# immaaane/dealii-stfem

Measured on AMD Instinct MI355X. Metric: space-time DoF/s per vmult (3D heat, Q4 space x cG(2) time); achieved HBM GB/s, higher is better.
Workload: dtype f64; 1 GPU; 3D heat, Q4 x cG(2), 72x72x72 cells Cartesian slab mesh, 48275138 space-time DoFs = BASELINE configs[1]; n_blocks=2, cells_per_gpu=373248, partition=z-slabs x1, kernel=st_sweep_pencil<f64>

## Files before the change

### dealii-stfem_amd/__init__.py

```python
import ctypes as C
import os
import subprocess

import numpy as np

_HERE = os.path.dirname(os.path.abspath(__file__))
LIB_PATH = os.path.join(_HERE, "libstfem_hip.so")
HEADER_PATH = os.path.join(os.path.dirname(_HERE), "include", "stfem.h")

CGP, DG = 0, 1


class StfemError(RuntimeError):
    def __init__(self, status, what=""):
        self.status = status
        msg = lib().stfem_strerror(status).decode()
        hip = lib().stfem_last_hip_error().decode()
        super().__init__(f"{what}: {msg} ({status})" + (f" [{hip}]" if hip else ""))


def build(force=False):
    args = ["make", "-C", os.path.join(_HERE, "csrc"), "-j8"]
    if force:
        args.append("-B")
# ... 127 lines not shown
                                        C.POINTER(_vp), _vp]),
    "stfem_stokes_st_vmult_slice_add": (C.c_int, [_vp, C.c_int, C.c_int, C.c_int, _dp, _dp, C.POINTER(_vp),
                                                  _vp, _vp, _vp]),
    "stfem_stokes_last_hip_error": (C.c_char_p, []),
    "stfem_stokes_set_weak_boundaries": (C.c_int, [_vp, C.c_int, C.c_int, C.c_double, C.c_double]),
    "stfem_stokes_n_face_points": (C.c_int64, [_vp]),
    "stfem_stokes_face_points": (C.c_int, [_vp, _dp]),
    "stfem_stokes_nitsche_rhs": (C.c_int, [_vp, _dp, _vp, _vp, _vp]),
    "stfem_stokes_pressure_ctx": (C.c_int, [_vp, C.POINTER(_vp)]),
    "stfem_stokes_pressure_mean_vectors": (C.c_int, [_vp, _dp, _dp, _dp]),
    "stfem_stokes_pressure_quadrature_points": (C.c_int, [_vp, C.c_int, _dp]),
    "stfem_stokes_pressure_difference": (C.c_int, [_vp, C.c_int, _vp, _dp, _dp, _vp]),
    "stfem_stokes_dgp_prolongate": (C.c_int, [_vp, _vp, _vp, _vp, C.c_int, _vp]),
    "stfem_stokes_dgp_restrict": (C.c_int, [_vp, _vp, _vp, _vp, C.c_int, _vp]),
    "stfem_stokes_vanka_create": (C.c_int, [_vp, C.c_int, C.POINTER(C.c_int32), _dp, _dp, C.POINTER(_vp)]),
    "stfem_stokes_vanka_destroy": (None, [_vp]),
    "stfem_stokes_vanka_n_classes": (C.c_int, [_vp]),
    "stfem_stokes_vanka_vmult": (C.c_int, [_vp, C.POINTER(_vp), C.POINTER(_vp), _vp]),
    "stfem_stokes_vanka_step": (C.c_int, [_vp, C.POINTER(_vp), C.c_double, C.c_int, C.POINTER(_vp), _vp]),
    "stfem_stokes_vanka_last_error": (C.c_char_p, []),
    "stfem_strerror": (C.c_char_p, [C.c_int]),
    "stfem_last_hip_error": (C.c_char_p, []),
    "stfem_last_kernel_name": (C.c_char_p, [_vp]),
}


def lib():
    global _lib
    if _lib is None:
        if not os.path.exists(LIB_PATH):
            raise ImportError(f"{LIB_PATH} is missing: run `make -C dealii-stfem_amd/csrc` "
                              "(or __graft_entry__.build()); there is no CPU fallback")
        L = C.CDLL(os.environ.get("STFEM_LIB", LIB_PATH))
        for name, (res, args) in SIGNATURES.items():
            f = getattr(L, name)
            f.restype = res
            f.argtypes = args
        _lib = L
    return _lib


def _p(a):
    return a.ctypes.data_as(_dp)


def _check(status, what):
# ... 170 lines not shown
               "stfem_space_vmult")

    def compute_diagonal(self, mass=None, laplace=None, stream=None):
        d = BlockVector(self, 1)
        _check(lib().stfem_diagonal(self._h,
                                    self.mass_matrix_scaling if mass is None else mass,
                                    self.laplace_matrix_scaling if laplace is None else laplace,
                                    d._h, stream), "stfem_diagonal")
        return d

    def get_matrix_diagonal(self, stream=None):
        return self.compute_diagonal(stream=stream)

    def get_matrix_diagonal_inverse(self, stream=None):
        d = BlockVector(self, 1)
        _check(lib().stfem_diagonal_inverse(self._h, self.mass_matrix_scaling, self.laplace_matrix_scaling,
                                            d._h, stream), "stfem_diagonal_inverse")
        return d

    @property
    def last_kernel_name(self):
        return lib().stfem_last_kernel_name(self._h).decode()


class PreconditionVanka:

    def __init__(self, ctx, Alpha, Beta, neighbour_mask=0, extended=None):
        self.ctx = ctx
        A = np.ascontiguousarray(Alpha, dtype=np.float64)
        B = np.ascontiguousarray(Beta, dtype=np.float64)
        assert A.shape == B.shape and A.shape[0] == A.shape[1]
        h = _vp()
        if extended is not None:
            _check(lib().stfem_vanka_create_partitioned_general(ctx._h, extended._h, A.shape[0], _p(A), _p(B), neighbour_mask, C.byref(h)),
                   "stfem_vanka_create_partitioned_general")
        else:
            _check(lib().stfem_vanka_create_partitioned(ctx._h, A.shape[0], _p(A), _p(B), neighbour_mask, C.byref(h)),
                   "stfem_vanka_create")
        self._h, self.n_blocks = h, A.shape[0]

    def __del__(self):
        if getattr(self, "_h", None) and _lib is not None:
            _lib.stfem_vanka_destroy(self._h)
            self._h = None

    @property
# ... 477 lines not shown
```

### dealii-stfem_amd/csrc/stfem_capi.hip

```cpp
#include "../../include/stfem.h"

#include "host_tables.h"
#include "stfem_internal.h"
#include "stfem_kernels.h"

#include <hip/hip_runtime.h>
#include <dlfcn.h>

#include <algorithm>
#include <cmath>
#include <cstdio>
#include <cstdlib>
#include <cstring>
#include <limits>
#include <new>
#include <string>
#include <vector>

using namespace stfem;

struct Prec64 {
  using real = double;
  using Sweep = f64::SweepParams;
  using Plan = f64::TilePlan;
// ... 150 lines not shown
    const double tol = 1e-13 * std::max({std::abs(up[0] - lo[0]), std::abs(up[1] - lo[1]),
                                         std::abs(up[2] - lo[2]), 1e-300});
    for (int64_t k = 0, o = 0; k < nvz && cart; ++k)
      for (int64_t j = 0; j < nvy && cart; ++j)
        for (int64_t i = 0; i < nvx; ++i, ++o) {
          if (std::abs(v[3 * o] - (lo[0] + c->h[0] * i)) > tol ||
              std::abs(v[3 * o + 1] - (lo[1] + c->h[1] * j)) > tol ||
              std::abs(v[3 * o + 2] - (lo[2] + c->h[2] * k)) > tol) {
            cart = false;
            break;
          }
        }
    c->cartesian = cart;
    c->vertices.assign(v, v + 3 * nv);
  }
  if (const char *v = getenv("STFEM_VARIANT")) c->variant = std::string(v) == "atomic" ? 1 : (std::string(v) == "tile" ? 2 : 0);
  auto env_int = [](const char *name, int dflt) { const char *e = getenv(name); return e ? atoi(e) : dflt; };
  c->env_tile_lz = env_int("STFEM_TILE_LZ", 0);
  c->env_exp = env_int("STFEM_EXP", 0);
  c->env_stagger = env_int("STFEM_STAGGER", 0);
  c->env_stagger_div = std::max(1, env_int("STFEM_STAGGER_DIV", 256));
  c->env_pencil_ty = env_int("STFEM_PENCIL_TY", 0);
  c->env_pencil_lz = env_int("STFEM_PENCIL_LZ", 0);
  c->env_timeline = getenv("STFEM_TIMELINE");
  if (hipMalloc(&c->d_scratch, sizeof(double) * (256 + 8 * 512)) != hipSuccess) {
    delete c;
    return STFEM_ERR_OUT_OF_MEMORY;
  }
  *out = c;
  return STFEM_OK;
}

void stfem_ctx_destroy(stfem_ctx *c)
{
  if (!c) return;
  (void)hipSetDevice(c->device);
  for (void *&p : c->d_coef)
    if (p) (void)hipFree(p);
  if (c->d_scratch) (void)hipFree(c->d_scratch);
  if (c->d_halo) (void)hipFree(c->d_halo);
  if (c->d_vertices) (void)hipFree(c->d_vertices);
  if (c->d_rule) (void)hipFree(c->d_rule);
  if (c->d_metric) (void)hipFree(c->d_metric);
  if (c->d_timeline) (void)hipFree(c->d_timeline);
  if (c->d_work) (void)hipFree(c->d_work);
  delete c;
}

int64_t stfem_n_dofs(const stfem_ctx *c) { return c ? c->ndofs : 0; }
int64_t stfem_n_cells(const stfem_ctx *c) { return c ? c->ncells : 0; }
int stfem_n_dofs_1d(const stfem_ctx *c, int32_t nd[3])
{
  if (!c || !nd) return STFEM_ERR_INVALID_ARGUMENT;
  for (int d = 0; d < 3; ++d) nd[d] = c->nd[d];
  return STFEM_OK;
}
int stfem_is_cartesian(const stfem_ctx *c) { return c && c->cartesian ? 1 : 0; }
int stfem_ctx_precision(const stfem_ctx *c) { return c ? c->prec : -1; }
const char *stfem_last_kernel_name(const stfem_ctx *c) { return c ? c->last_kernel : ""; }

int stfem_set_coefficient(stfem_ctx *c, int which, int layout, const double *host)
{
  if (!c || which < 0 || which > 1 || layout < 0 || layout > 2) return STFEM_ERR_INVALID_ARGUMENT;
  HIP_TRY(hipSetDevice(c->device));
  if (c->d_coef[which]) {
    HIP_TRY(hipFree(c->d_coef[which]));
    c->d_coef[which] = nullptr;
  }
// ... 162 lines not shown
  tp.nty = (c->nc[1] + tp.rows - 1) / tp.rows;
  const int ncz = c->nc[2];
  int ntc = 1;
  if (c->env_tile_lz > 0) {
    const int lz = std::max(1, std::min(ncz, c->env_tile_lz));
    ntc = (ncz + lz - 1) / lz;
  } else {
    (void)nbm;
    const int wpc = std::max(2, resident);
    const int64_t slots = int64_t(c->n_cu > 0 ? c->n_cu : 256) * wpc;
    const int64_t columns = int64_t((tp.ntx + 1) / 2) * tp.nty;
    double best = 1e300;
    for (int n = 1; n <= ncz; ++n) {
      const int64_t rounds = (columns * n + slots - 1) / slots;
      const double cost = double(rounds) * ((ncz + n - 1) / n + 1.0) * (1.0 + 1e-3 * n);
      if (cost < best) { best = cost; ntc = n; }
    }
  }
  tp.ntc = ntc;
  tp.lz = (ncz + ntc - 1) / ntc;
  tp.zp = c->p * tp.lz + 1;
}

template <class PL> static void plan_pencil(const stfem_ctx *c, PL &pp)
{
  pp.ntx = (c->nc[0] + pp.cpw - 2) / (pp.cpw - 1);
  const int cyw = pp.ty * 4;
  pp.ntyw = (c->nc[1] + cyw - 1) / cyw;
  const int ncz = c->nc[2];
  int B = c->env_pencil_lz > 0 ? c->env_pencil_lz : 8;
  B = std::max(B, (ncz + 47) / 48);
  int n = 0, r = ncz;
  pp.zb[0] = 0;
  while (r > 0) {
    const int sz = c->env_pencil_lz < 0 ? std::min(std::max(-c->env_pencil_lz, (ncz + 47) / 48), r)
                                        : std::min(B, std::max(1, (r + 2) / 3));
    r -= sz;
    pp.zb[n + 1] = pp.zb[n] + sz;
    if (n == 62 && r > 0) {
      pp.zb[n + 2] = ncz;
      n += 2;
      r = 0;
      break;
    }
    ++n;
  }
  pp.ntc = n;
  pp.lz = 0;
  for (int q = 0; q < n; ++q) pp.lz = std::max(pp.lz, pp.zb[q + 1] - pp.zb[q]);
  pp.zp = c->p * pp.lz + 1;
}

template <class PR> static int ensure_metric(stfem_ctx *c, bool use_lap, bool use_mass, hipStream_t st)
{
  using real = typename PR::real;
  const int n = c->p + 1;
  const size_t nm = size_t(c->ncells) * 8 * n * n * n;
  const int flags = (use_lap ? 1 : 0) | (use_mass ? 2 : 0);
  if (c->metric_valid && c->metric_flags == flags) return STFEM_OK;
  if (!c->d_vertices) {
    std::vector<double> v = c->vertices;
    if (v.empty()) {
      v.resize(size_t(c->nc[0] + 1) * (c->nc[1] + 1) * (c->nc[2] + 1) * 3);
      size_t o = 0;
      for (int k = 0; k <= c->nc[2]; ++k)
        for (int j = 0; j <= c->nc[1]; ++j)
          for (int i = 0; i <= c->nc[0]; ++i, ++o) {
            v[3 * o] = c->lower[0] + c->h[0] * i;
            v[3 * o + 1] = c->lower[1] + c->h[1] * j;
            v[3 * o + 2] = c->lower[2] + c->h[2] * k;
          }
    }
    std::vector<double> rule(c->tab.xq);
// ... 91 lines not shown
    for (int i0 = 0; i0 < nbi; i0 += panel) {
      const int tj = std::min(panel, nbo - j0), ti = std::min(panel, nbi - i0);
      bool nonzero = false;
      for (int j = 0; j < tj; ++j)
        for (int i = 0; i < ti; ++i) {
          prm.alpha[j * ti + i] = real(a[size_t(j0 + j) * nbi + i0 + i]);
          prm.beta[j * ti + i] = real(b[size_t(j0 + j) * nbi + i0 + i]);
          nonzero = nonzero || prm.alpha[j * ti + i] != real(0) || prm.beta[j * ti + i] != real(0);
        }
      const bool last_panel = i0 + panel >= nbi;
      if (!nonzero && (atomic || add || !first || !last_panel)) continue;
      prm.nbo = tj;
      prm.nbi = ti;
      for (int j = 0; j < tj; ++j) prm.dst[j] = static_cast<real *>(dst->blk[j0 + j]);
      for (int i = 0; i < ti; ++i) prm.src[i] = static_cast<const real *>(src->blk[i0 + i]);
      int rc;
      typename PR::PPlan pp;
      std::memset(&pp, 0, sizeof(pp));
      const int pencil_ty = c->env_pencil_ty;
      if (atomic) {
        rc = PR::atomic(c->p, prm, st);
        c->last_kernel = PR::atomic_name();
      } else if (c->variant == 0 && !general && PR::pencil_geometry(c->p, std::max(tj, ti), pencil_ty, pp) == 0) {
        plan_pencil(c, pp);
        const int nbm = std::max(tj, ti);
        const int nbm_r = nbm <= 4 ? nbm : (nbm <= 6 ? 6 : 8);
        const size_t ntiles = size_t(pp.ntx) * pp.ntyw * pp.ntc;
        const size_t nyh = ntiles * nbm_r * pp.zp * pp.tX, nzh = ntiles * nbm_r * pp.tYW * pp.tX;
        if (nyh + nzh > c->halo_doubles) {
          HIP_TRY(hipStreamSynchronize(st));
          if (c->d_halo) HIP_TRY(hipFree(c->d_halo));
          c->d_halo = nullptr;
          c->halo_doubles = 0;
          if (hipMalloc(&c->d_halo, (nyh + nzh) * sizeof(real)) != hipSuccess) return STFEM_ERR_OUT_OF_MEMORY;
          c->halo_doubles = nyh + nzh;
        }
        pp.yh = static_cast<real *>(c->d_halo);
        pp.zh = pp.yh + nyh;
        pp.add = (add || !first) ? 1 : 0;
        prm.gp = nullptr;
        if constexpr (sizeof(real) == 8) {
          if (c->grad_p && c->p == 2 && tj == 3 && ti == 3 && !pp.add && last_panel && !prm.coef_lap && !prm.coef_mass) {
            prm.gp = c->grad_p;
            prm.gscale = c->grad_scale;
            std::memcpy(prm.gw, c->grad_w, sizeof(prm.gw));
            c->grad_applied = true;
          }
        }
        if (!c->d_work) {
          if (hipMalloc(&c->d_work, 8 * 32 * sizeof(int)) != hipSuccess) return STFEM_ERR_OUT_OF_MEMORY;
          HIP_TRY(hipMemsetAsync(c->d_work, 0, 8 * 32 * sizeof(int), st));
        }
        pp.work = c->d_work;
        pp.grid = 2 * (c->n_cu > 0 ? c->n_cu : 256);
        const size_t ptl_n = ntiles * 4 * pp.lz * pp.ty * 8;
        if (c->env_timeline) {
          if (c->tl_n < ptl_n) {
            if (c->d_timeline) HIP_TRY(hipFree(c->d_timeline));
            c->d_timeline = nullptr;
            if (hipMalloc(&c->d_timeline, ptl_n * sizeof(long long)) != hipSuccess) return STFEM_ERR_OUT_OF_MEMORY;
            c->tl_n = ptl_n;
          }
          HIP_TRY(hipMemsetAsync(c->d_timeline, 0, ptl_n * sizeof(long long), st));
          pp.timeline = c->d_timeline;
        }
        rc = PR::pencil(c->p, prm, pp, st);
        c->last_kernel = PR::pencil_name();
        if (c->env_timeline && rc == 0) {
          HIP_TRY(hipStreamSynchronize(st));
          std::vector<long long> h(ptl_n);
          HIP_TRY(hipMemcpy(h.data(), c->d_timeline, ptl_n * sizeof(long long), hipMemcpyDeviceToHost));
          if (FILE *f = fopen(c->env_timeline, "wb")) {
            const long long hdr[4] = {(long long)ntiles, 4, (long long)pp.lz * pp.ty, 8};
            fwrite(hdr, sizeof(long long), 4, f);
            fwrite(h.data(), sizeof(long long), ptl_n, f);
            fclose(f);
          }
// ... 691 lines not shown
```

### dealii-stfem_amd/csrc/stfem_internal.h

```cpp
#pragma once
#include "../../include/stfem.h"

#include "host_tables.h"

#include <cstdint>
#include <vector>

struct stfem_ctx {
  int p = 0, device = 0, n_cu = 0;
  int nc[3] = {0, 0, 0}, nd[3] = {0, 0, 0};
  int64_t ndofs = 0, ncells = 0;
  int dmask = 0;
  bool cartesian = false;
  double lower[3] = {0, 0, 0}, h[3] = {1, 1, 1};
  stfem::ShapeTables tab;
  std::vector<double> vertices;
  int prec = 0;
  size_t es = sizeof(double);
  void *d_coef[2] = {nullptr, nullptr};
  int coef_layout[2] = {0, 0};
  double *d_scratch = nullptr;
  const char *last_kernel = "";
  void *d_halo = nullptr;
  size_t halo_doubles = 0;
  int variant = 0;
  int env_tile_lz = 0, env_exp = 0, env_stagger = 0, env_stagger_div = 256, env_pencil_ty = 0, env_pencil_lz = 0;
  const char *env_timeline = nullptr;
  int *d_work = nullptr;
  long long *d_timeline = nullptr;
  size_t tl_n = 0;
  double *d_vertices = nullptr, *d_rule = nullptr;
  void *d_metric = nullptr;
  bool metric_valid = false;
  int metric_flags = -1;
  const double *grad_p = nullptr;
  double grad_w[3][2][3][2];
  double grad_scale = 0.0;
  bool grad_applied = false;
};
int stfem_internal_set_gradient(stfem_ctx *c, const double *p, const double (*w)[2][3][2], double scale);

struct stfem_vec {
  stfem_ctx *ctx = nullptr;
  int device = 0;
  int nb = 0;
  bool owns = false;
  std::vector<void *> blk;
};


int stfem_internal_metric(stfem_ctx *c, const void **metric, void *stream);
// ... 9 lines not shown
```

### dealii-stfem_amd/csrc/stfem_kernels_decl.h

```cpp
namespace stfem {
namespace STFEM_NS {

using real_t = STFEM_REAL;

struct SweepParams {
  const real_t *src[MAX_BLOCKS];
  real_t *dst[MAX_BLOCKS];
  real_t alpha[MAX_BLOCKS * MAX_BLOCKS];
  real_t beta[MAX_BLOCKS * MAX_BLOCKS];
  int nbi, nbo;
  int ncx, ncy, ncz;
  int nx, ny, nz;
  int64_t ncells;
  int dmask;
  real_t vol;
  real_t ihx2, ihy2, ihz2;
  const real_t *coef_lap;
  const real_t *coef_mass;
  int experiment;
  real_t eo_Si[EO_N], eo_L[EO_N];
  real_t fd_W[EO_N], fd_lx[8], fd_ly[8], fd_lz[8];
  real_t eo_S[EO_N], eo_Dq[EO_N], eo_DqT[EO_N];
  const real_t *metric;
  const real_t *gp;
  real_t gw[3][2][3][2];
  real_t gscale;
};

struct TilePlan {
  int cw, rows;
  int wx;
  int ntx, nty, ntc;
  int lz;
  int tX, tY, zp;
  real_t *yh, *zh;
  real_t *xl, *xr;
  int add;
  int xcolor;
  int stagger;
  int stagger_div;
  int experiment;
  long long *timeline;
};

struct PencilPlan {
  int cpw, ty;
  int ntx, ntyw, ntc;
  int lz;
  int zb[65];
  int tX, tYW, zp;
  real_t *yh, *zh;
  int add;
  int *work;
  int grid;
  long long *timeline;
};
int pencil_geometry(int p, int nbm, int ty, PencilPlan &plan);
int launch_pencil(int p, const SweepParams &prm, const PencilPlan &plan, void *stream);

int launch_cart_atomic(int p, const SweepParams &prm, void *stream);
const char *cart_atomic_name(int p, int nbm);

struct DiagParams {
  real_t *diag;
  int ncx, ncy, ncz, nx, ny, p, dmask;
  real_t ms, ls;
  real_t vol, ihx2, ihy2, ihz2;
  const real_t *coef_lap, *coef_mass;
  const real_t *metric;
  real_t m1[8], l1[8];
  real_t S[64], D[64];
};
// ... 13 lines not shown
```

### dealii-stfem_amd/csrc/stfem_pencil.hip

```cpp
#include "stfem_core.h"

#include <cstdio>
#include <cstdlib>

#ifndef STFEM_PENCIL_P
#define STFEM_PENCIL_P 0
#endif

namespace stfem {
namespace STFEM_PREC {

namespace {

constexpr int PENCIL_WY = 4;

#ifndef STFEM_PENCIL_EXP
#define STFEM_PENCIL_EXP 0
#endif
constexpr int PEX = STFEM_PENCIL_EXP;

template <typename T> __device__ __forceinline__ void vm_load(T &dst, const T *p)
{
  if constexpr (sizeof(T) == 8) asm volatile("global_load_dwordx2 %0, %1, off" : "=v"(dst) : "v"(p) : "memory");
  else asm volatile("global_load_dword %0, %1, off" : "=v"(dst) : "v"(p) : "memory");
// ... 69 lines not shown
  const int wave = __builtin_amdgcn_readfirstlane(threadIdx.x >> 6);
  real_t *lds = smem + wave * Core::LDS_PER_WAVE;
  real_t *mail_base = smem + WY * Core::LDS_PER_WAVE;
  real_t *mail_out = mail_base + wave * 2 * PG::MAIL;
  const real_t *mail_in = mail_base + (wave - 1) * 2 * PG::MAIL;
  volatile int *flags = reinterpret_cast<volatile int *>(mail_base + (WY - 1) * 2 * PG::MAIL);
  volatile int *prod = flags, *cons = flags + WY;
  volatile int *s_tile = flags + 2 * WY;
  real_t *wtab = const_cast<real_t *>(reinterpret_cast<volatile real_t *>(flags + 2 * WY + 4));
  [[maybe_unused]] real_t *gpt = wtab + PG::WTAB + wave * PG::GPT_WAVE;
  if constexpr (PG::WLDS) {
    for (int e = threadIdx.x; e < NBM * NBM; e += PG::NT) {
      const int j = e / NBM, q = e % NBM;
      const bool ok = j < prm.nbo && q < prm.nbi;
      wtab[2 * e] = ok ? prm.alpha[j * prm.nbi + q] * prm.vol : real_t(0);
      wtab[2 * e + 1] = ok ? prm.beta[j * prm.nbi + q] * prm.vol : real_t(0);
    }
  }
  auto flag_wait = [&](volatile int *f, int target) {
    while (*f < target) __builtin_amdgcn_s_sleep(1);
    asm volatile("" ::: "memory");
  };

  const int ncol = pp.ntx * pp.ntyw;
  unsigned xcc = 0;
  asm volatile("s_getreg_b32 %0, hwreg(HW_REG_XCC_ID)" : "=s"(xcc));
  xcc &= 7;
  for (;;) {
  __syncthreads();
  if (threadIdx.x == 0) {
    int t = -1;
    const int per = ncol / 8, rem = ncol % 8;
    for (int q = 0; q < 8 && t < 0; ++q) {
      const int x = (xcc + q) & 7;
      const int lo = x * per + min(x, rem), n = per + (x < rem ? 1 : 0);
      if (n > 0) {
        const int k = atomicAdd(pp.work + 32 * x, 1);
        if (k < n * pp.ntc) t = (k / n) * ncol + lo + k % n;
      }
    }
    *s_tile = t;
  }
  prod[wave] = 0;
  cons[wave] = 0;
  __syncthreads();
  const int id = __builtin_amdgcn_readfirstlane(*s_tile);
  if (id < 0) break;
  const int tx = id % pp.ntx, tyw = (id / pp.ntx) % pp.ntyw, tc = id / (pp.ntx * pp.ntyw);
  const int wg_tile = id;
  const int wy = tyw * WY + wave;
  const int cx0 = tx * (CPW - 1) - 1, cy0 = wy * TY;
  const int cz0 = pp.zb[tc];
  const int nlay = pp.zb[tc + 1] - cz0;
  const int nslot = min(CPW, prm.ncx - cx0);
  const int ncy_t = max(0, min(TY, prm.ncy - cy0));
  const bool last_x = tx == pp.ntx - 1, last_z = tc == pp.ntc - 1;
  const bool mesh_top = cy0 + TY >= prm.ncy;
  const bool top_mail = !mesh_top && wave < WY - 1;
  const bool top_halo = !mesh_top && wave == WY - 1;
  const bool has_lower = wave > 0;

  const bool lane_ok = lane < PG::ACTIVE;
  const int l = lane_ok ? lane : 0;
  const int i = l % N, c = (l / N) % CPW, blk = l / (N * CPW);
  const int X = P * c + i;
  unsigned lf = 0;
  {
    const bool cell_ok = lane_ok && c < nslot && cx0 + c >= 0 && ncy_t > 0;
    const int cxl = cx0 + (cell_ok ? c : 1);
    const bool out = cell_ok && blk < prm.nbo;
    const bool st = out && c > 0 && (i < P || cxl == prm.ncx - 1);
    const bool xcon = ((prm.dmask & 1) && cxl == 0 && i == 0) || ((prm.dmask & 2) && cxl == prm.ncx - 1 && i == P);
    lf = (cell_ok && blk < prm.nbi ? LF_IN : 0) | (out ? LF_OUT : 0) | (c == nslot - 1 ? LF_LAST : 0) |
         (st ? LF_ST : 0) | (xcon ? LF_XCON : 0);
  }
  const int cx = cx0 + ((lf & (LF_IN | LF_OUT)) ? c : 1);

  [[maybe_unused]] real_t gwx[3] = {real_t(0), real_t(0), real_t(0)}, gWy[N][2], gWz[N][2];
  [[maybe_unused]] int gxv = 0;
// ... 351 lines not shown
    flag_wait(prod + (wave - 1), nlay);
    const real_t *m = mail_in + ((nlay - 1) & 1) * PG::MAIL + lane;
    real_t *d = dst_lane + plane_stride * (int64_t(P) * (nlay - 1));
    real_t v[N];
    STFEM_UNROLL
    for (int z = 0; z < P; ++z) v[z] = pend[z] + m[64 * z];
    v[P] = zfin0 + m[64 * P];
    if (lf & LF_ST) {
      const bool xc = lf & LF_XCON;
      STFEM_UNROLL
      for (int z = 0; z < P; ++z) put(d + plane_stride * z, xc ? real_t(0) : v[z]);
      if (last_z) put(d + plane_stride * P, xc ? real_t(0) : v[P]);
      else (pp.zh + ((int64_t(wg_tile) * NBM + blk) * pp.tYW + P * TY * wave) * pp.tX + X)[0] = xc ? real_t(0) : v[P];
    }
  }
  }
}

template <int P>
__global__ __launch_bounds__(256) void st_pencil_fixup(const SweepParams prm, const PencilPlan pp, int nbm, int cpw, int ty)
{
  const int id = blockIdx.x;
  if (id == 0 && blockIdx.y == 0 && blockIdx.z == 0 && threadIdx.x < 8) pp.work[32 * threadIdx.x] = 0;
  const int tx = id % pp.ntx, tyw = (id / pp.ntx) % pp.ntyw, tc = id / (pp.ntx * pp.ntyw);
  const int has_y = tyw > 0, has_z = tc > 0;
  if (!(has_y | has_z)) return;
  const int cyw = ty * PENCIL_WY;
  const int cx0 = tx * (cpw - 1) - 1, cy0 = tyw * cyw, cz0 = pp.zb[tc];
  const int nslot = min(cpw, prm.ncx - cx0), ncy_t = min(cyw, prm.ncy - cy0);
  const int nlay = pp.zb[tc + 1] - cz0;
  const bool last_x = tx == pp.ntx - 1, last_y = tyw == pp.ntyw - 1, last_z = tc == pp.ntc - 1;
  const int x_begin = P, x_end = P * nslot + (last_x ? 1 : 0);
  const int Yn = P * ncy_t + (last_y ? 1 : 0), Zn = P * nlay + (last_z ? 1 : 0);
  const int lpr = pp.tX <= 16 ? 16 : (pp.tX <= 32 ? 32 : 64), nrg = 256 / lpr;
  const int X = threadIdx.x % lpr, rg = threadIdx.x / lpr;
  if (X < x_begin || X >= x_end) return;
  const int64_t plane_stride = int64_t(prm.nx) * prm.ny;
  const int64_t g0 = int64_t(P) * cx0 + X + int64_t(prm.nx) * (int64_t(P) * cy0) + plane_stride * (int64_t(P) * cz0);
  const int tid_y = id - pp.ntx, tid_z = id - pp.ntx * pp.ntyw, tid_yz = tid_z - pp.ntx;
  const int top_below = has_z ? P * (cz0 - pp.zb[tc - 1]) : 0;
  const int j = blockIdx.y;
  real_t *d = prm.dst[j] + g0;
  const int64_t sy = int64_t(pp.zp) * pp.tX, sz = int64_t(pp.tYW) * pp.tX;
  const real_t *yh_y = pp.yh + (int64_t(tid_y) * nbm + j) * sy + X;
  const real_t *yh_yz = pp.yh + (int64_t(tid_yz) * nbm + j) * sy + X;
  const real_t *zh_z = pp.zh + (int64_t(tid_z) * nbm + j) * sz + X;
  constexpr int U = 4;
  if (has_y && blockIdx.z == 0)
    for (int Z0 = rg + has_z; Z0 < Zn; Z0 += U * nrg) {
      real_t s[U], v[U];
      STFEM_UNROLL
      for (int u = 0; u < U; ++u) {
        const int Z = Z0 + u * nrg;
        s[u] = v[u] = real_t(0);
        if (Z < Zn) {
          s[u] = yh_y[Z * pp.tX];
          v[u] = d[plane_stride * Z];
        }
      }
      STFEM_UNROLL
      for (int u = 0; u < U; ++u) {
        const int Z = Z0 + u * nrg;
        if (Z < Zn) d[plane_stride * Z] = v[u] + s[u];
      }
    }
  if (has_z && blockIdx.z == 1)
    for (int Y0 = rg; Y0 < Yn; Y0 += U * nrg) {
      real_t s[U], v[U];
      STFEM_UNROLL
      for (int u = 0; u < U; ++u) {
        const int Y = Y0 + u * nrg;
        s[u] = v[u] = real_t(0);
        if (Y < Yn) {
          s[u] = zh_z[Y * pp.tX];
          if (Y == 0 && has_y) s[u] += yh_y[0] + yh_yz[top_below * pp.tX];
          v[u] = d[int64_t(prm.nx) * Y];
        }
      }
      STFEM_UNROLL
      for (int u = 0; u < U; ++u) {
        const int Y = Y0 + u * nrg;
        if (Y < Yn) d[int64_t(prm.nx) * Y] = v[u] + s[u];
      }
    }
}

template <int P, int NBM, int TY> int launch_pencil_ty(const SweepParams &prm, const PencilPlan &pp, hipStream_t st)
{
  using PG = PencilGeom<P, NBM, TY>;
  (void)hipGetLastError();
  const bool coef = prm.coef_lap || prm.coef_mass;
  const int nblocks = pp.ntx * pp.ntyw * pp.ntc;
  const int grid = nblocks < pp.grid ? nblocks : pp.grid;
#define STFEM_LAUNCH(AA, CC)                                                                                       \
  do {                                                                                                            \
    static bool lds_set = false;                                                                                  \
    if (!lds_set) {                                                                                               \
      if (hipFuncSetAttribute(reinterpret_cast<const void *>(&st_sweep_pencil<P, NBM, TY, AA, CC>),               \
                              hipFuncAttributeMaxDynamicSharedMemorySize, int(PG::LDS_BYTES)) != hipSuccess)      \
        return -3;                                                                                                \
      lds_set = true;                                                                                             \
    }                                                                                                             \
    hipLaunchKernelGGL((st_sweep_pencil<P, NBM, TY, AA, CC>), dim3(grid), dim3(PG::NT), PG::LDS_BYTES, st, prm, pp); \
  } while (0)
  if constexpr (PG::HAS_GRAD) {
    if (prm.gp) {
      if (pp.add || coef) return -2;
      static bool lds_set = false;
      if (!lds_set) {
        if (hipFuncSetAttribute(reinterpret_cast<const void *>(&st_sweep_pencil<P, NBM, TY, false, false, true>), hipFuncAttributeMaxDynamicSharedMemorySize,
                                int(PG::LDS_BYTES)) != hipSuccess)
          return -3;
        lds_set = true;
      }
      hipLaunchKernelGGL((st_sweep_pencil<P, NBM, TY, false, false, true>), dim3(grid), dim3(PG::NT), PG::LDS_BYTES, st, prm, pp);
    }
  }
  if (PG::HAS_GRAD && prm.gp) {
  } else if (pp.add && coef) STFEM_LAUNCH(true, true);
  else if (pp.add) STFEM_LAUNCH(true, false);
  else if (coef) STFEM_LAUNCH(false, true);
  else STFEM_LAUNCH(false, false);
#undef STFEM_LAUNCH
  const bool sweep_ok = hipGetLastError() == hipSuccess;
  bool fixed_up = false;
  if (sweep_ok && (pp.ntyw > 1 || pp.ntc > 1)) {
    hipLaunchKernelGGL((st_pencil_fixup<P>), dim3(nblocks, prm.nbo, 2), dim3(256), 0, st, prm, pp, NBM, PG::CPW, TY);
    fixed_up = hipGetLastError() == hipSuccess;
    if (!fixed_up) (void)hipMemsetAsync(pp.work, 0, 8 * 32 * sizeof(int), st);
    return fixed_up ? 0 : -3;
  }
  if (hipMemsetAsync(pp.work, 0, 8 * 32 * sizeof(int), st) != hipSuccess || !sweep_ok) return -3;
  return 0;
}

constexpr int pencil_ty(int p, int nbm) { return (p == 4 && nbm == 3) ? 1 : ((p <= 2 && nbm <= 4) ? 4 : 2); }
constexpr int pencil_ty_default(int p, int nbm) { return pencil_ty(p, nbm); }

template <int P, int NBM> int launch_pencil_t(const SweepParams &prm, const PencilPlan &pp, hipStream_t st)
{
  if constexpr (Geometry<P, NBM>::CELLS_PER_WAVE < 2) return -2;
  else {
    if (pp.ty == 1) return launch_pencil_ty<P, NBM, 1>(prm, pp, st);
    if constexpr (pencil_ty(P, NBM) >= 2)
      if (pp.ty == 2) return launch_pencil_ty<P, NBM, 2>(prm, pp, st);
    if constexpr (pencil_ty(P, NBM) >= 4)
      if (pp.ty == 4) return launch_pencil_ty<P, NBM, 4>(prm, pp, st);
    return -2;
  }
// ... 56 lines not shown
```

### include/stfem.h

```cpp
#ifndef STFEM_H
#define STFEM_H

#include <stddef.h>
#include <stdint.h>

#ifdef __cplusplus
extern "C" {
#endif

typedef enum {
  STFEM_OK = 0,
  STFEM_ERR_INVALID_ARGUMENT = -1,
  STFEM_ERR_UNSUPPORTED = -2,
  STFEM_ERR_HIP = -3,
  STFEM_ERR_NO_DEVICE = -4,
  STFEM_ERR_SHAPE_MISMATCH = -5,
  STFEM_ERR_ALIAS = -6,
  STFEM_ERR_OUT_OF_MEMORY = -7,
  STFEM_ERR_COMM = -8
} stfem_status;

typedef struct stfem_ctx stfem_ctx;
typedef struct stfem_vec stfem_vec;

// ... 178 lines not shown
const char *stfem_stokes_last_hip_error(void);

int stfem_stokes_pressure_ctx(stfem_stokes_ctx *ctx, stfem_ctx **out);
int stfem_stokes_pressure_mean_vectors(stfem_stokes_ctx *ctx, double *ones, double *weights, double *volume);
int stfem_stokes_pressure_quadrature_points(const stfem_stokes_ctx *ctx, int nq, double *out);
int stfem_stokes_pressure_difference(stfem_stokes_ctx *ctx, int nq, const double *p, const double *exact_at_points, double out[2], void *stream);
int stfem_stokes_dgp_prolongate(stfem_stokes_ctx *fine, stfem_stokes_ctx *coarse, double *dst_fine, const double *src_coarse, int add, void *stream);
int stfem_stokes_dgp_restrict(stfem_stokes_ctx *fine, stfem_stokes_ctx *coarse, double *dst_coarse, const double *src_fine, int add, void *stream);

typedef struct stfem_stokes_vanka stfem_stokes_vanka;
int stfem_stokes_vanka_create(stfem_stokes_ctx *ctx, int n_blocks, const int32_t *block_variable, const double *Alpha, const double *Beta,
                              stfem_stokes_vanka **out);
void stfem_stokes_vanka_destroy(stfem_stokes_vanka *v);
int stfem_stokes_vanka_n_classes(const stfem_stokes_vanka *v);
int stfem_stokes_vanka_vmult(stfem_stokes_vanka *v, double *const *dst_blocks, const double *const *src_blocks, void *stream);
int stfem_stokes_vanka_step(stfem_stokes_vanka *v, double *const *dst_blocks, double omega, int accumulate, const double *const *src_blocks,
                            void *stream);
const char *stfem_stokes_vanka_last_error(void);

const char *stfem_strerror(int status);
const char *stfem_last_hip_error(void);
void stfem_trace_push(const char *name);
void stfem_trace_pop(void);
const char *stfem_last_kernel_name(const stfem_ctx *ctx);

#ifdef __cplusplus
}
#endif
#endif
```

Measured before the change: 166.2 billion space-time DoF/s.

## Schedule pencil sweep via precomputed piece table with gang-based z partitioning

Replaces the fixed column-by-z-chunk pencil decomposition with a host-built, device-cached table of pieces. Each piece records its column, z range and its neighbours below and in y. When the grid is large relative to the column count, rows (tyw, z) are split into gangs so each XCC queue gets balanced, variable-length z pieces ordered by round. The sweep kernel and the fixup kernel read piece records from the table, and the fixup walks neighbour links to find y-halo rows across mismatched z boundaries. This aims to improve load balance and occupancy across XCDs, at the cost of extra indirection and pointer chasing in the fixup kernel.

Result: slower. 157.9 billion space-time DoF/s (-5.0%).

```diff
diff --git a/dealii-stfem_amd/__init__.py b/dealii-stfem_amd/__init__.py
--- a/dealii-stfem_amd/__init__.py
+++ b/dealii-stfem_amd/__init__.py
@@ -173,6 +173,7 @@
     "stfem_strerror": (C.c_char_p, [C.c_int]),
     "stfem_last_hip_error": (C.c_char_p, []),
     "stfem_last_kernel_name": (C.c_char_p, [_vp]),
+    "stfem_pencil_plan": (C.c_int, [_vp, C.c_int, C.POINTER(C.c_int32), C.c_int, C.POINTER(C.c_int32)]),
 }
 
 
@@ -389,6 +390,15 @@
     def last_kernel_name(self):
         return lib().stfem_last_kernel_name(self._h).decode()
 
+    def pencil_plan(self, n_blocks):
+        info = (C.c_int32 * 4)()
+        n = lib().stfem_pencil_plan(self._h, n_blocks, None, 0, info)
+        if n < 0:
+            raise StfemError(n, "stfem_pencil_plan")
+        out = np.zeros((n, 8), dtype=np.int32)
+        _check(min(0, lib().stfem_pencil_plan(self._h, n_blocks, out.ctypes.data_as(C.POINTER(C.c_int32)), n, info)), "stfem_pencil_plan")
+        return out, dict(zip(("cpw", "ty", "gangs", "grid"), (int(v) for v in info)))
+
 
 class PreconditionVanka:
 
diff --git a/dealii-stfem_amd/csrc/stfem_capi.hip b/dealii-stfem_amd/csrc/stfem_capi.hip
--- a/dealii-stfem_amd/csrc/stfem_capi.hip
+++ b/dealii-stfem_amd/csrc/stfem_capi.hip
@@ -196,6 +196,7 @@
   c->env_stagger_div = std::max(1, env_int("STFEM_STAGGER_DIV", 256));
   c->env_pencil_ty = env_int("STFEM_PENCIL_TY", 0);
   c->env_pencil_lz = env_int("STFEM_PENCIL_LZ", 0);
+  c->env_pencil_gangs = env_int("STFEM_PENCIL_GANGS", 0);
   c->env_timeline = getenv("STFEM_TIMELINE");
   if (hipMalloc(&c->d_scratch, sizeof(double) * (256 + 8 * 512)) != hipSuccess) {
     delete c;
@@ -218,6 +219,8 @@
   if (c->d_metric) (void)hipFree(c->d_metric);
   if (c->d_timeline) (void)hipFree(c->d_timeline);
   if (c->d_work) (void)hipFree(c->d_work);
+  for (auto &t : c->pencil_tables)
+    if (t.d) (void)hipFree(t.d);
   delete c;
 }
 
@@ -426,33 +429,143 @@
   tp.zp = c->p * tp.lz + 1;
 }
 
-template <class PL> static void plan_pencil(const stfem_ctx *c, PL &pp)
-{
-  pp.ntx = (c->nc[0] + pp.cpw - 2) / (pp.cpw - 1);
-  const int cyw = pp.ty * 4;
-  pp.ntyw = (c->nc[1] + cyw - 1) / cyw;
+static int plan_pencil_pieces(const stfem_ctx *c, int cpw, int ty, int grid, stfem_ctx::PencilTable &t)
+{
+  const int ntx = (c->nc[0] + cpw - 2) / (cpw - 1);
+  const int cyw = ty * 4;
+  const int ntyw = (c->nc[1] + cyw - 1) / cyw;
   const int ncz = c->nc[2];
-  int B = c->env_pencil_lz > 0 ? c->env_pencil_lz : 8;
-  B = std::max(B, (ncz + 47) / 48);
-  int n = 0, r = ncz;
-  pp.zb[0] = 0;
-  while (r > 0) {
-    const int sz = c->env_pencil_lz < 0 ? std::min(std::max(-c->env_pencil_lz, (ncz + 47) / 48), r)
-                                        : std::min(B, std::max(1, (r + 2) / 3));
-    r -= sz;
-    pp.zb[n + 1] = pp.zb[n] + sz;
-    if (n == 62 && r > 0) {
-      pp.zb[n + 2] = ncz;
-      n += 2;
-      r = 0;
-      break;
-    }
-    ++n;
-  }
-  pp.ntc = n;
-  pp.lz = 0;
-  for (int q = 0; q < n; ++q) pp.lz = std::max(pp.lz, pp.zb[q + 1] - pp.zb[q]);
-  pp.zp = c->p * pp.lz + 1;
+  if (ntx >= 65536 || ntyw >= 32768 || ncz >= (1 << 30)) return -1;
+  struct Piece { int tx, tyw, z0, n, round; };
+  std::vector<Piece> list[8];
+
+  std::vector<int> zb(1, 0);
+  {
+    int B = c->env_pencil_lz > 0 ? c->env_pencil_lz : 8;
+    B = std::max(B, (ncz + 47) / 48);
+    int r = ncz;
+    while (r > 0) {
+      const int sz = c->env_pencil_lz < 0 ? std::min(std::max(-c->env_pencil_lz, (ncz + 47) / 48), r)
+                                          : std::min(B, std::max(1, (r + 2) / 3));
+      r -= sz;
+      zb.push_back(zb.back() + sz);
+    }
+  }
+  const int64_t ncol = int64_t(ntx) * ntyw, rows = int64_t(ntyw) * ncz;
+  const int slots = std::max(1, grid / 8);
+  int64_t gangs = 0;
+  if (c->env_pencil_gangs > 0) gangs = std::min<int64_t>(c->env_pencil_gangs, rows);
+  else if (c->env_pencil_lz == 0) {
+    const int g = slots / ntx;
+    if (g >= 1 && 8 * g * ntx >= 7 * slots && 8 * int64_t(g) <= rows && ncol * int64_t(zb.size() - 1) > grid) gangs = 8 * int64_t(g);
+  }
+  if (gangs > 0) {
+    std::vector<int> part(8, 0);
+    for (int64_t i = 0; i < gangs; ++i) {
+      const int x = int(i * 8 / gangs);
+      int64_t lo = i * rows / gangs;
+      const int64_t hi = (i + 1) * rows / gangs;
+      int round = 0;
+      while (lo < hi) {
+        const int tyw = int(lo / ncz), z0 = int(lo % ncz);
+        const int n = int(std::min<int64_t>(hi - lo, ncz - z0));
+        for (int tx = 0; tx < ntx; ++tx) list[x].push_back({tx, tyw, z0, n, round});
+        lo += n;
+        ++round;
+      }
+    }
+    for (auto &l : list)
+      std::stable_sort(l.begin(), l.end(), [](const Piece &a, const Piece &b) { return a.round < b.round; });
+  } else {
+    const int64_t per = ncol / 8, rem = ncol % 8;
+    for (int x = 0; x < 8; ++x) {
+      const int64_t lo = x * per + std::min<int64_t>(x, rem), n = per + (x < rem ? 1 : 0);
+      for (size_t tc = 0; tc + 1 < zb.size(); ++tc)
+        for (int64_t col = lo; col < lo + n; ++col) list[x].push_back({int(col % ntx), int(col / ntx), zb[tc], zb[tc + 1] - zb[tc], 0});
+    }
+  }
+
+  t.ntx = ntx;
+  t.ntyw = ntyw;
+  t.gangs = int(gangs);
+  t.lz = 0;
+  t.host.clear();
+  int id = 0;
+  std::vector<std::vector<std::pair<int, int>>> column{size_t(ncol)};
+  for (int x = 0; x < 8; ++x) {
+    t.xb[x] = id;
+    for (const Piece &q : list[x]) {
+      const int rec[8] = {q.tx, q.tyw, q.z0, q.n, -1, -1, -1, q.z0 + q.n == ncz ? 1 : 0};
+      t.host.insert(t.host.end(), rec, rec + 8);
+      column[size_t(q.tyw) * ntx + q.tx].push_back({q.z0, id});
+      t.lz = std::max(t.lz, q.n);
+      ++id;
+    }
+  }
+  t.xb[8] = t.npieces = id;
+  for (auto &col : column) std::sort(col.begin(), col.end());
+  for (int tyw = 0; tyw < ntyw; ++tyw)
+    for (int tx = 0; tx < ntx; ++tx) {
+      const auto &col = column[size_t(tyw) * ntx + tx];
+      for (size_t k = 0; k < col.size(); ++k) {
+        int *rec = &t.host[size_t(col[k].second) * 8];
+        if (k > 0) rec[4] = col[k - 1].second;
+        if (k + 1 < col.size()) rec[5] = col[k + 1].second;
+        if (tyw > 0) {
+          const auto &low = column[size_t(tyw - 1) * ntx + tx];
+          size_t m = 0;
+          while (m + 1 < low.size() && low[m + 1].first <= col[k].first) ++m;
+          rec[6] = low[m].second;
+        }
+      }
+    }
+  return 0;
+}
+
+static int pencil_table(stfem_ctx *c, int cpw, int ty, int grid, bool upload, const stfem_ctx::PencilTable **out)
+{
+  for (auto &t : c->pencil_tables)
+    if (t.cpw == cpw && t.ty == ty && t.grid == grid) {
+      if (upload && !t.d) {
+        if (hipMalloc(&t.d, t.host.size() * sizeof(int)) != hipSuccess) return STFEM_ERR_OUT_OF_MEMORY;
+        HIP_TRY(hipMemcpy(t.d, t.host.data(), t.host.size() * sizeof(int), hipMemcpyHostToDevice));
+      }
+      *out = &t;
+      return STFEM_OK;
+    }
+  stfem_ctx::PencilTable t;
+  t.cpw = cpw;
+  t.ty = ty;
+  t.grid = grid;
+  if (plan_pencil_pieces(c, cpw, ty, grid, t) != 0) return STFEM_ERR_UNSUPPORTED;
+  c->pencil_tables.push_back(std::move(t));
+  return pencil_table(c, cpw, ty, grid, upload, out);
+}
+
+static int pencil_grid(const stfem_ctx *c) { return 2 * (c->n_cu > 0 ? c->n_cu : 256); }
+
+extern "C" int stfem_pencil_plan(stfem_ctx *c, int n_blocks, int32_t *pieces, int capacity, int32_t info[4])
+{
+  if (!c || n_blocks < 1 || n_blocks > MAX_BLOCKS) return STFEM_ERR_INVALID_ARGUMENT;
+  stfem::f64::PencilPlan p64;
+  stfem::f32::PencilPlan p32;
+  std::memset(&p64, 0, sizeof(p64));
+  std::memset(&p32, 0, sizeof(p32));
+  if (c->variant != 0 || !c->cartesian || c->p > 4) return STFEM_ERR_UNSUPPORTED;
+  const int rc = c->prec ? stfem::f32::pencil_geometry(c->p, n_blocks, c->env_pencil_ty, p32) : stfem::f64::pencil_geometry(c->p, n_blocks, c->env_pencil_ty, p64);
+  if (rc != 0) return STFEM_ERR_UNSUPPORTED;
+  const stfem_ctx::PencilTable *t = nullptr;
+  const int st = pencil_table(c, c->prec ? p32.cpw : p64.cpw, c->prec ? p32.ty : p64.ty, pencil_grid(c), false, &t);
+  if (st != STFEM_OK) return st;
+  if (pieces)
+    for (int i = 0; i < std::min(capacity, t->npieces) * 8; ++i) pieces[i] = t->host[size_t(i)];
+  if (info) {
+    info[0] = t->cpw;
+    info[1] = t->ty;
+    info[2] = t->gangs;
+    info[3] = t->grid;
+  }
+  return t->npieces;
 }
 
 template <class PR> static int ensure_metric(stfem_ctx *c, bool use_lap, bool use_mass, hipStream_t st)
@@ -590,10 +703,20 @@
         rc = PR::atomic(c->p, prm, st);
         c->last_kernel = PR::atomic_name();
       } else if (c->variant == 0 && !general && PR::pencil_geometry(c->p, std::max(tj, ti), pencil_ty, pp) == 0) {
-        plan_pencil(c, pp);
+        pp.grid = pencil_grid(c);
+        const stfem_ctx::PencilTable *pt = nullptr;
+        const int prc = pencil_table(c, pp.cpw, pp.ty, pp.grid, true, &pt);
+        if (prc != STFEM_OK) return prc;
+        pp.ntx = pt->ntx;
+        pp.ntyw = pt->ntyw;
+        pp.npieces = pt->npieces;
+        pp.lz = pt->lz;
+        pp.zp = c->p * pp.lz + 1;
+        for (int x = 0; x <= 8; ++x) pp.xb[x] = pt->xb[x];
+        pp.pieces = pt->d;
         const int nbm = std::max(tj, ti);
         const int nbm_r = nbm <= 4 ? nbm : (nbm <= 6 ? 6 : 8);
-        const size_t ntiles = size_t(pp.ntx) * pp.ntyw * pp.ntc;
+        const size_t ntiles = size_t(pp.npieces);
         const size_t nyh = ntiles * nbm_r * pp.zp * pp.tX, nzh = ntiles * nbm_r * pp.tYW * pp.tX;
         if (nyh + nzh > c->halo_doubles) {
           HIP_TRY(hipStreamSynchronize(st));
@@ -620,7 +743,6 @@
           HIP_TRY(hipMemsetAsync(c->d_work, 0, 8 * 32 * sizeof(int), st));
         }
         pp.work = c->d_work;
-        pp.grid = 2 * (c->n_cu > 0 ? c->n_cu : 256);
         const size_t ptl_n = ntiles * 4 * pp.lz * pp.ty * 8;
         if (c->env_timeline) {
           if (c->tl_n < ptl_n) {
diff --git a/dealii-stfem_amd/csrc/stfem_internal.h b/dealii-stfem_amd/csrc/stfem_internal.h
--- a/dealii-stfem_amd/csrc/stfem_internal.h
+++ b/dealii-stfem_amd/csrc/stfem_internal.h
@@ -24,9 +24,16 @@
   void *d_halo = nullptr;
   size_t halo_doubles = 0;
   int variant = 0;
-  int env_tile_lz = 0, env_exp = 0, env_stagger = 0, env_stagger_div = 256, env_pencil_ty = 0, env_pencil_lz = 0;
+  int env_tile_lz = 0, env_exp = 0, env_stagger = 0, env_stagger_div = 256, env_pencil_ty = 0, env_pencil_lz = 0, env_pencil_gangs = 0;
   const char *env_timeline = nullptr;
   int *d_work = nullptr;
+  struct PencilTable {
+    int cpw = 0, ty = 0, grid = 0;
+    int ntx = 0, ntyw = 0, npieces = 0, lz = 0, gangs = 0, xb[9] = {0, 0, 0, 0, 0, 0, 0, 0, 0};
+    std::vector<int> host;
+    int *d = nullptr;
+  };
+  std::vector<PencilTable> pencil_tables;
   long long *d_timeline = nullptr;
   size_t tl_n = 0;
   double *d_vertices = nullptr, *d_rule = nullptr;
diff --git a/dealii-stfem_amd/csrc/stfem_kernels_decl.h b/dealii-stfem_amd/csrc/stfem_kernels_decl.h
--- a/dealii-stfem_amd/csrc/stfem_kernels_decl.h
+++ b/dealii-stfem_amd/csrc/stfem_kernels_decl.h
@@ -43,11 +43,14 @@
   long long *timeline;
 };
 
+constexpr int PENCIL_PIECE_INTS = 8;
 struct PencilPlan {
   int cpw, ty;
-  int ntx, ntyw, ntc;
+  int ntx, ntyw;
+  int npieces;
   int lz;
-  int zb[65];
+  int xb[9];
+  const int *pieces;
   int tX, tYW, zp;
   real_t *yh, *zh;
   int add;
diff --git a/dealii-stfem_amd/csrc/stfem_pencil.hip b/dealii-stfem_amd/csrc/stfem_pencil.hip
--- a/dealii-stfem_amd/csrc/stfem_pencil.hip
+++ b/dealii-stfem_amd/csrc/stfem_pencil.hip
@@ -115,7 +115,6 @@
     asm volatile("" ::: "memory");
   };
 
-  const int ncol = pp.ntx * pp.ntyw;
   unsigned xcc = 0;
   asm volatile("s_getreg_b32 %0, hwreg(HW_REG_XCC_ID)" : "=s"(xcc));
   xcc &= 7;
@@ -123,31 +122,37 @@
   __syncthreads();
   if (threadIdx.x == 0) {
     int t = -1;
-    const int per = ncol / 8, rem = ncol % 8;
     for (int q = 0; q < 8 && t < 0; ++q) {
       const int x = (xcc + q) & 7;
-      const int lo = x * per + min(x, rem), n = per + (x < rem ? 1 : 0);
+      const int lo = pp.xb[x], n = pp.xb[x + 1] - lo;
       if (n > 0) {
         const int k = atomicAdd(pp.work + 32 * x, 1);
-        if (k < n * pp.ntc) t = (k / n) * ncol + lo + k % n;
-      }
-    }
-    *s_tile = t;
+        if (k < n) t = lo + k;
+      }
+    }
+    s_tile[0] = t;
+    if (t >= 0) {
+      const int *e = pp.pieces + PENCIL_PIECE_INTS * t;
+      s_tile[1] = e[0] | (e[1] << 16);
+      s_tile[2] = e[2];
+      s_tile[3] = e[3] | ((e[7] & 1) << 30);
+    }
   }
   prod[wave] = 0;
   cons[wave] = 0;
   __syncthreads();
-  const int id = __builtin_amdgcn_readfirstlane(*s_tile);
+  const int id = __builtin_amdgcn_readfirstlane(s_tile[0]);
   if (id < 0) break;
-  const int tx = id % pp.ntx, tyw = (id / pp.ntx) % pp.ntyw, tc = id / (pp.ntx * pp.ntyw);
+  const int e_col = __builtin_amdgcn_readfirstlane(s_tile[1]), e_lay = __builtin_amdgcn_readfirstlane(s_tile[3]);
+  const int tx = e_col & 0xffff, tyw = e_col >> 16;
   const int wg_tile = id;
   const int wy = tyw * WY + wave;
   const int cx0 = tx * (CPW - 1) - 1, cy0 = wy * TY;
-  const int cz0 = pp.zb[tc];
-  const int nlay = pp.zb[tc + 1] - cz0;
+  const int cz0 = __builtin_amdgcn_readfirstlane(s_tile[2]);
+  const int nlay = e_lay & 0x3fffffff;
   const int nslot = min(CPW, prm.ncx - cx0);
   const int ncy_t = max(0, min(TY, prm.ncy - cy0));
-  const bool last_x = tx == pp.ntx - 1, last_z = tc == pp.ntc - 1;
+  const bool last_x = tx == pp.ntx - 1, last_z = (e_lay >> 30) & 1;
   const bool mesh_top = cy0 + TY >= prm.ncy;
   const bool top_mail = !mesh_top && wave < WY - 1;
   const bool top_halo = !mesh_top && wave == WY - 1;
@@ -545,14 +550,14 @@
 {
   const int id = blockIdx.x;
   if (id == 0 && blockIdx.y == 0 && blockIdx.z == 0 && threadIdx.x < 8) pp.work[32 * threadIdx.x] = 0;
-  const int tx = id % pp.ntx, tyw = (id / pp.ntx) % pp.ntyw, tc = id / (pp.ntx * pp.ntyw);
-  const int has_y = tyw > 0, has_z = tc > 0;
+  const int *e = pp.pieces + PENCIL_PIECE_INTS * id;
+  const int tx = e[0], tyw = e[1], cz0 = e[2], nlay = e[3], below = e[4], ylow = e[6];
+  const int has_y = tyw > 0, has_z = below >= 0;
   if (!(has_y | has_z)) return;
   const int cyw = ty * PENCIL_WY;
-  const int cx0 = tx * (cpw - 1) - 1, cy0 = tyw * cyw, cz0 = pp.zb[tc];
+  const int cx0 = tx * (cpw - 1) - 1, cy0 = tyw * cyw;
   const int nslot = min(cpw, prm.ncx - cx0), ncy_t = min(cyw, prm.ncy - cy0);
-  const int nlay = pp.zb[tc + 1] - cz0;
-  const bool last_x = tx == pp.ntx - 1, last_y = tyw == pp.ntyw - 1, last_z = tc == pp.ntc - 1;
+  const bool last_x = tx == pp.ntx - 1, last_y = tyw == pp.ntyw - 1, last_z = e[7] & 1;
   const int x_begin = P, x_end = P * nslot + (last_x ? 1 : 0);
   const int Yn = P * ncy_t + (last_y ? 1 : 0), Zn = P * nlay + (last_z ? 1 : 0);
   const int lpr = pp.tX <= 16 ? 16 : (pp.tX <= 32 ? 32 : 64), nrg = 256 / lpr;
@@ -560,52 +565,70 @@
   if (X < x_begin || X >= x_end) return;
   const int64_t plane_stride = int64_t(prm.nx) * prm.ny;
   const int64_t g0 = int64_t(P) * cx0 + X + int64_t(prm.nx) * (int64_t(P) * cy0) + plane_stride * (int64_t(P) * cz0);
-  const int tid_y = id - pp.ntx, tid_z = id - pp.ntx * pp.ntyw, tid_yz = tid_z - pp.ntx;
-  const int top_below = has_z ? P * (cz0 - pp.zb[tc - 1]) : 0;
   const int j = blockIdx.y;
   real_t *d = prm.dst[j] + g0;
   const int64_t sy = int64_t(pp.zp) * pp.tX, sz = int64_t(pp.tYW) * pp.tX;
-  const real_t *yh_y = pp.yh + (int64_t(tid_y) * nbm + j) * sy + X;
-  const real_t *yh_yz = pp.yh + (int64_t(tid_yz) * nbm + j) * sy + X;
-  const real_t *zh_z = pp.zh + (int64_t(tid_z) * nbm + j) * sz + X;
+  const real_t *yh_j = pp.yh + int64_t(j) * sy + X, *zero = nullptr;
+  auto y_rows = [&](int gz, const real_t *&lo, const real_t *&up) {
+    int r = ylow;
+    const int *q = pp.pieces + PENCIL_PIECE_INTS * r;
+    while (gz >= P * (q[2] + q[3]) && q[5] >= 0) {
+      r = q[5];
+      q = pp.pieces + PENCIL_PIECE_INTS * r;
+    }
+    const int zl = gz - P * q[2];
+    up = yh_j + int64_t(r) * nbm * sy + int64_t(zl) * pp.tX;
+    lo = zero;
+    if (zl == 0 && q[4] >= 0) lo = yh_j + int64_t(q[4]) * nbm * sy + int64_t(P * pp.pieces[PENCIL_PIECE_INTS * q[4] + 3]) * pp.tX;
+  };
   constexpr int U = 4;
   if (has_y && blockIdx.z == 0)
     for (int Z0 = rg + has_z; Z0 < Zn; Z0 += U * nrg) {
-      real_t s[U], v[U];
+      real_t sl[U], su[U], v[U];
       STFEM_UNROLL
       for (int u = 0; u < U; ++u) {
         const int Z = Z0 + u * nrg;
-        s[u] = v[u] = real_t(0);
+        sl[u] = su[u] = v[u] = real_t(0);
         if (Z < Zn) {
-          s[u] = yh_y[Z * pp.tX];
+          const real_t *lo, *up;
+          y_rows(P * cz0 + Z, lo, up);
+          if (lo) sl[u] = *lo;
+          su[u] = *up;
           v[u] = d[plane_stride * Z];
         }
       }
       STFEM_UNROLL
       for (int u = 0; u < U; ++u) {
         const int Z = Z0 + u * nrg;
-        if (Z < Zn) d[plane_stride * Z] = v[u] + s[u];
-      }
-    }
-  if (has_z && blockIdx.z == 1)
+        if (Z < Zn) d[plane_stride * Z] = (v[u] + sl[u]) + su[u];
+      }
+    }
+  if (has_z && blockIdx.z == 1) {
+    const real_t *zh_z = pp.zh + (int64_t(below) * nbm + j) * sz + X;
     for (int Y0 = rg; Y0 < Yn; Y0 += U * nrg) {
-      real_t s[U], v[U];
+      real_t s[U], sl[U], su[U], v[U];
       STFEM_UNROLL
       for (int u = 0; u < U; ++u) {
         const int Y = Y0 + u * nrg;
-        s[u] = v[u] = real_t(0);
+        s[u] = sl[u] = su[u] = v[u] = real_t(0);
         if (Y < Yn) {
           s[u] = zh_z[Y * pp.tX];
-          if (Y == 0 && has_y) s[u] += yh_y[0] + yh_yz[top_below * pp.tX];
+          if (Y == 0 && has_y) {
+            const real_t *lo, *up;
+            y_rows(P * cz0, lo, up);
+            if (lo) sl[u] = *lo;
+            su[u] = *up;
+          }
           v[u] = d[int64_t(prm.nx) * Y];
         }
       }
       STFEM_UNROLL
       for (int u = 0; u < U; ++u) {
         const int Y = Y0 + u * nrg;
-        if (Y < Yn) d[int64_t(prm.nx) * Y] = v[u] + s[u];
-      }
-    }
+        if (Y < Yn) d[int64_t(prm.nx) * Y] = ((v[u] + s[u]) + sl[u]) + su[u];
+      }
+    }
+  }
 }
 
 template <int P, int NBM, int TY> int launch_pencil_ty(const SweepParams &prm, const PencilPlan &pp, hipStream_t st)
@@ -613,7 +636,7 @@
   using PG = PencilGeom<P, NBM, TY>;
   (void)hipGetLastError();
   const bool coef = prm.coef_lap || prm.coef_mass;
-  const int nblocks = pp.ntx * pp.ntyw * pp.ntc;
+  const int nblocks = pp.npieces;
   const int grid = nblocks < pp.grid ? nblocks : pp.grid;
 #define STFEM_LAUNCH(AA, CC)                                                                                       \
   do {                                                                                                            \
@@ -647,7 +670,7 @@
 #undef STFEM_LAUNCH
   const bool sweep_ok = hipGetLastError() == hipSuccess;
   bool fixed_up = false;
-  if (sweep_ok && (pp.ntyw > 1 || pp.ntc > 1)) {
+  if (sweep_ok && pp.npieces > pp.ntx) {
     hipLaunchKernelGGL((st_pencil_fixup<P>), dim3(nblocks, prm.nbo, 2), dim3(256), 0, st, prm, pp, NBM, PG::CPW, TY);
     fixed_up = hipGetLastError() == hipSuccess;
     if (!fixed_up) (void)hipMemsetAsync(pp.work, 0, 8 * 32 * sizeof(int), st);
diff --git a/include/stfem.h b/include/stfem.h
--- a/include/stfem.h
+++ b/include/stfem.h
@@ -224,6 +224,7 @@
 const char *stfem_last_hip_error(void);
 void stfem_trace_push(const char *name);
 void stfem_trace_pop(void);
+int stfem_pencil_plan(stfem_ctx *ctx, int n_blocks, int32_t *pieces, int capacity, int32_t info[4]);
 const char *stfem_last_kernel_name(const stfem_ctx *ctx);
 
 #ifdef __cplusplus
```
